# ydixon/yolo_v3

Measured on AMD Instinct MI355X. Metric: images/sec (YOLOv3 forward + decode + NMS, 416x416, bs=64 per GPU), higher is better.
Workload: dtype f32 (exact fp32 MFMA); 1 GPU; 416x416 bs=64 per GPU, 64 distinct synthetic scenes per GPU, SW-1 synthetic weights, conf=0.50 nms=0.40; global_batch=64, parallelism=dp1, entry=Detector.run_device, lanes=2

## Files before the change

### yolo_v3_amd/_ffi.py

```python
import ctypes
import os

_HERE = os.path.dirname(os.path.abspath(__file__))
LIB_PATH = (os.environ.get("YV3_LIB") if os.environ.get("YV3_MEASURE") == "1" else None) or os.path.join(_HERE, "libyv3.so")

if os.environ.get("YV3_MEASURE") != "1":
    _stray = sorted(k for k in os.environ if k.startswith("YV3_") and k not in ("YV3_MEASURE", "YV3_DIST_BACKEND", "YV3_DUMP_PLAN"))
    if _stray:
        import warnings
        warnings.warn("yolo_v3_amd: %s set but ignored -- library / kernel-selection overrides are honoured in measurement sessions only "
                      "(YV3_MEASURE=1); the bundled libyv3.so and the default plans are used" % ", ".join(_stray), RuntimeWarning)

F32, BF16, F32X3, F32H2 = 0, 1, 2, 3
BF16_ACT = 4
F16 = 5
I8 = 6
ACT_LINEAR, ACT_LEAKY = 0, 1
PP_EVAL, PP_PROB = 1, 2
OPT_NO_PINGPONG, OPT_K3S1, OPT_WINO_EVEN, OPT_WINO_ALWAYS, OPT_TWO_LANES, OPT_WINO4_TILES = 1, 2, 4, 8, 16, 32
OPT_TILE_SHIFT = 8
(TILE_AUTO, TILE_256x128_W8, TILE_128x128_W8, TILE_128x128_W4, TILE_128x64, TILE_256x128_W4, TILE_256x256, TILE_256x128_W4_ROLL,
 TILE_256x256_ROLL, TILE_256x256_ROLL4) = range(10)
TILE_192x256_ROLL, TILE_W4_192x128, TILE_256x256_PP3, TILE_256x256_PP4, TILE_192x256_PP3, TILE_192x256_PP4 = 11, 12, 13, 14, 15, 16
T0_F32_TILE_64, T0_F32_TILE_128_W4, T0_F32_TILE_128_1X1, T0_WINO2_HALF, T0_WINO2_FULL = 2, 6, 7, 8, 9
T0_WINO4_NEVER, T0_WINO4_ALWAYS, T0_GEMM_NEVER, T0_GEMM_ALWAYS = 10, 11, 13, 14
T1_WINO4_NO_EVEN, T1_WINO4_NO_FULL, T1_GEMM_ALL_ROWS = 1, 2, 3
T1P_NO_SHORT_K, T1P_WINO_OTHER_LOOP, T1P_BF16_ROUND3, T1P_BF16_NO_192, T1P_NO_W4 = 1, 2, 8, 16, 32
T1P_NO_W4_1X1, T1P_NO_W4_3X3, T1P_W4_LANES_3X3, T1P_BF16_ROLL, T1P_BF16_PP3 = 64, 128, 256, 512, 1024
KERNEL_LINE_BYTES = 96


def conv2d_kernel(desc):
    buf = ctypes.create_string_buffer(KERNEL_LINE_BYTES)
    check(lib().yv3_conv2d_kernel(ctypes.byref(desc), buf, KERNEL_LINE_BYTES), "yv3_conv2d_kernel")
    return buf.value.decode()

c_void_p, c_int, c_float, c_size_t, c_longlong = (ctypes.c_void_p, ctypes.c_int, ctypes.c_float,
                                                  ctypes.c_size_t, ctypes.c_longlong)


class ConvDesc(ctypes.Structure):
    _fields_ = [("x", c_void_p), ("x2", c_void_p), ("w", c_void_p), ("alpha", c_void_p), ("beta", c_void_p),
                ("residual", c_void_p), ("y", c_void_p),
                ("B", c_int), ("H", c_int), ("W", c_int), ("cin", c_int), ("cin_up", c_int),
                ("cout", c_int), ("cout_pad", c_int), ("k", c_int), ("stride", c_int), ("act", c_int),
                ("dtype", c_int), ("out_dtype", c_int), ("flags", c_void_p),
                ("workspace", c_void_p), ("workspace_bytes", ctypes.c_size_t),
                ("dec_out", c_void_p), ("dec_out_batch_stride", c_longlong), ("dec_stride", c_float),
                ("dec_anchors", c_float * 6), ("options", ctypes.c_uint), ("big_tile_min", c_int), ("tune", c_int * 4),
                ("x_plane_stride", c_longlong), ("x2_plane_stride", c_longlong), ("y_plane_stride", c_longlong),
                ("w_wino", c_void_p), ("alpha_wino", c_void_p), ("wino_ws", c_void_p), ("wino_ws_bytes", ctypes.c_size_t),
                ("w_wino4", c_void_p), ("s_res", c_float), ("inv_s_out", c_float)]


COCO_MAX_MAXDETS = 8
ELIMIT = -6


class CocoEvalDesc(ctypes.Structure):
    _fields_ = [("n_gt", c_int), ("n_det", c_int), ("n_img", c_int), ("n_cat", c_int),
                ("gt_img", c_void_p), ("gt_cat", c_void_p), ("gt_box", c_void_p), ("gt_area", c_void_p),
                ("gt_crowd", c_void_p), ("gt_id", c_void_p),
                ("det_img", c_void_p), ("det_cat", c_void_p), ("det_box", c_void_p), ("det_score", c_void_p),
                ("n_iou", c_int), ("n_rec", c_int), ("n_area", c_int), ("n_maxdet", c_int),
                ("iou_thrs", c_void_p), ("rec_thrs", c_void_p), ("area_rng", c_void_p),
                ("max_dets", c_int * COCO_MAX_MAXDETS),
                ("precision", c_void_p), ("recall", c_void_p), ("scores", c_void_p), ("status", c_void_p)]


YOLO_LOSS_MAX_ROWS = 1024
EINVAL, ESHAPE, EWORKSPACE = -1, -2, -3


class YoloLossDesc(ctypes.Structure):
    _fields_ = [("logits", c_void_p), ("grad", c_void_p),
                ("stride_b", c_longlong), ("stride_p", c_longlong), ("stride_c", c_longlong),
                ("target", c_void_p), ("B", c_int), ("H", c_int), ("W", c_int), ("T", c_int), ("num_class", c_int),
                ("img_dim_h", c_float), ("anchors", c_float * 18), ("mask", c_int * 3),
                ("sums", c_void_p), ("counts", c_void_p), ("status", c_void_p)]
# ... 163 lines not shown
```

### yolo_v3_amd/csrc/conv_select.cpp

```cpp
#include "conv_select.h"
#include <stdio.h>

yv3_conv_shape yv3_conv_out_shape(const yv3_conv_desc* d) {
    const int pad = (d->k - 1) / 2;
    yv3_conv_shape s;
    s.Ho = (d->H + 2 * pad - d->k) / d->stride + 1;
    s.Wo = (d->W + 2 * pad - d->k) / d->stride + 1;
    s.M = (long long)d->B * s.Ho * s.Wo;
    return s;
}


static bool planes_wino_rule(const yv3_conv_desc* d, int np, long long ncu) {
    const int npad = d->cout_pad;
    const bool k3 = d->k == 3, dual = d->cin_up > 0, out_f32 = d->out_dtype == YV3_F32;
    if (!(d->w_wino && np == 2 && k3 && d->stride == 1 && !out_f32 && !dual && d->alpha_wino && npad % 128 == 0 &&
          d->x_plane_stride <= 0 && d->y_plane_stride <= 0)) return false;
    const long long tiles = (((long long)d->B * ((d->H + 1) / 2) * ((d->W + 1) / 2) + 127) / 128) * (npad / 128);
    if (d->options & YV3_OPT_WINO_ALWAYS) return true;
#ifndef YV3_AB_NO_TWO_LANES_RULE
    if (d->options & YV3_OPT_TWO_LANES) return tiles * 100 >= 27 * ncu;
#endif
    if (tiles * 100 <= 105 * ncu) return tiles * 100 >= 62 * ncu;
    return tiles * 100 >= 75 * ((tiles + ncu - 1) / ncu) * ncu;
// ... 125 lines not shown
    if (P > 1 && (8 * ((tail + 7) / 8) * P > YV3_SEL_WINO4_MAX_TAIL_WG || (lone_only && W > ncu))) return -1;
    const long long f = W <= ncu ? 1 : W <= 2 * ncu ? 2 : 2 * ((W + 2 * ncu - 1) / (2 * ncu));
    return (6 / P) * nkx * f + (P > 1 ? 29 + 5 * P : 0);
}
static void wino4_schedule(const yv3_conv_desc* d, long long items, int ncu, int* n_full, int* parts) {
    const int slots = 2 * ncu;
    *n_full = (int)items; *parts = 1;
    if ((d->options & YV3_OPT_WINO4_TILES) || d->tune[1] == YV3_T1_WINO4_NO_EVEN || items < 1) return;
    const long long full = d->tune[1] == YV3_T1_WINO4_NO_FULL ? 0 : (items / slots) * slots;
    const long long tail = items - full;
    if (tail == 0) return;
    const int nkx = 6 * (d->cin / 32);
    int best = 1; long long best_cost = wino4_tail_cost(tail, 1, nkx, ncu, false);
    for (int P = 2; P <= 6; ++P) {
        if (6 % P) continue;
        const long long cost = wino4_tail_cost(tail, P, nkx, ncu, full > 0);
        if (cost >= 0 && cost < best_cost) { best = P; best_cost = cost; }
    }
    if ((d->tune[2] == 2 || d->tune[2] == 3 || d->tune[2] == 6) && wino4_tail_cost(tail, d->tune[2], nkx, ncu, false) >= 0) best = d->tune[2];
    if (best == 1) return;
    *n_full = (int)full; *parts = best;
}

static bool wino4_pays(const yv3_conv_desc* d, long long items, long long ncu) {
    if ((d->options & YV3_OPT_WINO4_TILES) || d->tune[1] == YV3_T1_WINO4_NO_EVEN) return items * 10 >= 3 * ncu;
    return d->cin >= 256 ? true : d->cin == 128 ? items * 100 >= 17 * ncu : items * 100 >= 39 * ncu;
}

yv3_f32_choice yv3_select_f32(const yv3_conv_desc* d, int ncu_) {
    yv3_f32_choice c = {};
    c.form = YV3_FORM_DIRECT; c.launches = 1; c.parts = 1;
    const auto fail = [&c](int rc) { c.rc = rc; return c; };
    const auto pick = [&c](yv3_f32_kernel k, int ntiles) { c.kernel = k; c.ntiles = ntiles; return c; };
    const long long ncu = ncu_;
    const bool k3 = d->k == 3, dual = d->cin_up > 0;
    const int tune0 = d->tune[0];
    const yv3_conv_shape sh = yv3_conv_out_shape(d);
    const long long M = sh.M;
    if (M > 0x7fffffffLL) return fail(YV3_ESHAPE);
    c.Ho = sh.Ho; c.Wo = sh.Wo; c.M = (int)M;
    c.pin = !(d->options & YV3_OPT_TWO_LANES);

    if (d->w_wino4 && d->wino_ws && k3 && d->stride == 1 && !dual && d->cout % YV3_SEL_WINO4_CHANNELS == 0 && (d->cin == 64 || d->cin % 128 == 0) &&
        d->cout_pad == d->cout && d->alpha && tune0 != YV3_T0_WINO4_NEVER) {
        const long long T = (long long)d->B * ((d->H + 3) / 4) * ((d->W + 3) / 4);
        const long long items = ((T + YV3_SEL_WINO4_TILES - 1) / YV3_SEL_WINO4_TILES) * (d->cout / YV3_SEL_WINO4_CHANNELS);
        if ((d->options & YV3_OPT_WINO_ALWAYS) || tune0 == YV3_T0_WINO4_ALWAYS || wino4_pays(d, items, ncu)) {
            if (d->wino_ws_bytes < yv3_wino4_ws_bytes(d->B, d->H, d->W, d->cin)) return fail(YV3_EWORKSPACE);
            const unsigned long long vb = 36ull * T * d->cin * 4, ub = 36ull * d->cout * d->cin * 4;
            if (vb > 0xffffffffull || ub > 0xffffffffull) return fail(YV3_ESHAPE);
            if (items * 6 > 0x7fffffffLL) return fail(YV3_ESHAPE);
            c.form = YV3_FORM_WINOGRAD4; c.launches = 2;
            wino4_schedule(d, items, ncu_, &c.n_full, &c.parts);
            return pick(YV3_FK_WINO4, d->cout / YV3_SEL_WINO4_CHANNELS);
        }
    }

    if (d->w_wino && d->alpha_wino && k3 && d->stride == 1 && !dual && d->cout % 128 == 0 && d->cout_pad == d->cout) {
        const long long T2 = (long long)d->B * ((d->H + 1) / 2) * ((d->W + 1) / 2);
        const long long t128 = ((T2 + 127) / 128) * (d->cout / 128);
        if ((d->options & YV3_OPT_WINO_ALWAYS) || t128 * 100 >= 40 * ncu) {
            if (!d->wino_ws || d->wino_ws_bytes < (size_t)16 * T2 * d->cin * sizeof(float)) return fail(YV3_EWORKSPACE);
            c.form = YV3_FORM_WINOGRAD; c.launches = 2;
            const long long last = t128 % ncu;
            c.wino2_half = tune0 == YV3_T0_WINO2_HALF || (tune0 != YV3_T0_WINO2_FULL && ((t128 > ncu && last > 0 && 3 * last <= 2 * ncu) || 2 * t128 <= ncu));
            return pick(YV3_FK_WINO2, d->cout / 128);
        }
    }

    const int np = d->cout_pad;
    const bool g_k1 = d->k == 1 && d->stride == 1, g_k3 = k3 && d->cout % 128 == 0 && tune0 == YV3_T0_GEMM_ALWAYS;
    if ((g_k1 || g_k3) && !d->cin_up && !d->residual && d->cin % 32 == 0 && d->cout % 64 == 0 && d->cout <= 1024 && d->cout_pad == d->cout && tune0 != YV3_T0_GEMM_NEVER &&
        !((long long)d->B * d->H * d->W * d->cin * 4 > 0xfffffe00LL || M * d->cout * 4 > 0xffffffffLL || (long long)d->cout * d->cin * d->k * d->k * 4 > 0xffffffffLL)) {
        const bool wide = d->cout % 128 == 0;
        const int bm = (wide ? 2 : 4) * YV3_SEL_GEMM_WAVE_M, bn = (wide ? 4 : 2) * YV3_SEL_GEMM_WAVE_N, ntn = d->cout / bn;
        const long long mt = (M + bm - 1) / bm;
        if (tune0 == YV3_T0_GEMM_ALWAYS || mt * ntn >= ncu) {
            long long mt_run = mt;
            if (d->tune[1] != YV3_T1_GEMM_ALL_ROWS) {
                const long long rounds = mt * ntn / ncu, rest = mt * ntn - rounds * ncu;
                if (rounds >= 1 && rest > 0 && 2 * rest <= ncu) mt_run = rounds * ncu / ntn;
            }
            c.gemm_rows = (int)(mt_run * bm < M ? mt_run * bm : M);
            const long long tiles = ((c.gemm_rows + bm - 1) / bm) * ntn;
            c.gemm_grid = (int)(tiles < ncu ? (tiles + 7) / 8 * 8 : ncu);
            if (c.gemm_rows < M) {
                c.launches = 2;
                c.rest = k3 ? YV3_FK_128x128_W8 : np % 128 == 0 ? YV3_FK_64x64 : YV3_FK_128x64;
                c.rest_ntiles = k3 ? np / 128 : np / 64;
            }
            return pick(k3 ? YV3_FK_GEMM_K3 : wide ? YV3_FK_GEMM_128x128 : YV3_FK_GEMM_256x64, ntn);
        }
    }

    if (np % 128 == 0) {
        const long long blocks128 = ((M + 127) / 128) * (np / 128);
        if (blocks128 >= 384 && tune0 == YV3_T0_F32_TILE_128_W4) return pick(YV3_FK_128x128_W4, np / 128);
        if (blocks128 >= 384 && tune0 != YV3_T0_F32_TILE_64 && (k3 || tune0 == YV3_T0_F32_TILE_128_1X1)) return pick(YV3_FK_128x128_W8, np / 128);
        return pick(YV3_FK_64x64, np / 64);
    }
    if (np % 64 == 0) return pick(YV3_FK_128x64, np / 64);
    return pick(YV3_FK_128x32, np / 32);
}


const char* yv3_planes_kernel_name(yv3_planes_kernel k) {
// ... 58 lines not shown
```

### yolo_v3_amd/csrc/conv_select.h

```cpp
#pragma once
#include <stddef.h>
#include "yv3.h"

enum {
    YV3_TILE_AUTO = 0,
    YV3_TILE_256x128_W8 = 1,
    YV3_TILE_128x128_W8 = 2,
    YV3_TILE_128x128_W4 = 3,
    YV3_TILE_128x64 = 4,
    YV3_TILE_256x128_W4 = 5,
    YV3_TILE_256x256 = 6,
    YV3_TILE_256x128_W4_ROLL = 7,
    YV3_TILE_256x256_ROLL = 8,
    YV3_TILE_256x256_ROLL4 = 9,
    YV3_TILE_192x256_ROLL = 11,
    YV3_TILE_W4_192x128 = 12,
    YV3_TILE_256x256_PP3 = 13,
    YV3_TILE_256x256_PP4 = 14,
    YV3_TILE_192x256_PP3 = 15,
    YV3_TILE_192x256_PP4 = 16,
};
enum {
    YV3_T0_F32_TILE_64 = 2,
    YV3_T0_F32_TILE_128_W4 = 6,
    YV3_T0_F32_TILE_128_1X1 = 7,
    YV3_T0_WINO2_HALF = 8,
    YV3_T0_WINO2_FULL = 9,
    YV3_T0_WINO4_NEVER = 10,
    YV3_T0_WINO4_ALWAYS = 11,
    YV3_T0_GEMM_NEVER = 13,
    YV3_T0_GEMM_ALWAYS = 14,
};
enum {
    YV3_T1_WINO4_NO_EVEN = 1,
    YV3_T1_WINO4_NO_FULL = 2,
    YV3_T1_GEMM_ALL_ROWS = 3,
};
enum {
    YV3_T1P_NO_SHORT_K = 1,
    YV3_T1P_WINO_OTHER_LOOP = 2,
    YV3_T1P_BF16_ROUND3 = 8,
    YV3_T1P_BF16_NO_192 = 16,
    YV3_T1P_NO_W4 = 32,
    YV3_T1P_NO_W4_1X1 = 64,
    YV3_T1P_NO_W4_3X3 = 128,
    YV3_T1P_W4_LANES_3X3 = 256,
    YV3_T1P_BF16_ROLL = 512,
    YV3_T1P_BF16_PP3 = 1024,
};

constexpr int YV3_SEL_CHUNK = 32;
constexpr int YV3_SEL_W4_BM = 192, YV3_SEL_W4_BN = 128;
constexpr int YV3_SEL_GEMM_WAVE_M = 64, YV3_SEL_GEMM_WAVE_N = 32;
constexpr int YV3_SEL_WINO4_TILES = 32, YV3_SEL_WINO4_CHANNELS = 64;

#define YV3_SK_MAX_WG 512
#define YV3_SK_PART_BYTES (512 * 64 * 4)
static inline size_t yv3_sk_bytes() { return (size_t)YV3_SK_MAX_WG * (YV3_SK_PART_BYTES + sizeof(int)); }
#define YV3_WINO_SK_MAX_WG 512
#define YV3_WINO_SK_PART_BYTES (512 * 128 * 4)
static inline size_t yv3_wino_sk_bytes() { return (size_t)YV3_WINO_SK_MAX_WG * (YV3_WINO_SK_PART_BYTES + sizeof(int)) + 256; }
constexpr int YV3_SEL_WINO4_MAX_TAIL_WG = 2 * YV3_WINO_SK_MAX_WG - 1;
static inline size_t yv3_wino4_v_bytes(int B, int H, int W, int cin) { return (size_t)36 * B * ((H + 3) / 4) * ((W + 3) / 4) * cin * sizeof(float); }
static inline size_t yv3_wino4_ws_bytes(int B, int H, int W, int cin) { return ((yv3_wino4_v_bytes(B, H, W, cin) + 255) & ~(size_t)255) + yv3_wino_sk_bytes(); }

enum yv3_planes_kernel {
    YV3_PK_256x128_W8,
    YV3_PK_128x128_W8,
    YV3_PK_128x128_W4,
    YV3_PK_128x64,
    YV3_PK_128x32,
    YV3_PK_256x128_W8_PP6,
    YV3_PK_256x128_W4,
    YV3_PK_256x128_W4_ROLL,
    YV3_PK_256x256,
    YV3_PK_256x256_ROLL,
    YV3_PK_256x256_ROLL4,
    YV3_PK_256x256_PP3,
    YV3_PK_256x256_PP4,
    YV3_PK_192x256_ROLL,
    YV3_PK_192x256_PP3,
    YV3_PK_192x256_PP4,
    YV3_PK_W4_192x128,
    YV3_PK_K3S1_256x128,
    YV3_PK_K3S1_128x128,
    YV3_PK_K3S1_128x64,
    YV3_PK_WINO_PINGPONG,
    YV3_PK_WINO_ROLL,
    YV3_PK_WINO_EVEN,
};
const char* yv3_planes_kernel_name(yv3_planes_kernel k);
enum yv3_planes_loop {
    YV3_LOOP_PLAIN,
    YV3_LOOP_ROLLING,
    YV3_LOOP_PINGPONG,
};
const char* yv3_planes_loop_name(yv3_planes_loop l);
struct yv3_planes_choice {
    int rc;
    int form, launches;
    yv3_planes_kernel kernel;
    int Ho, Wo, M;
    int ntiles;
    yv3_planes_loop loop;
    bool stream_k;
    int grid;
};

enum yv3_f32_kernel {
    YV3_FK_NONE,
    YV3_FK_128x128_W8, YV3_FK_128x128_W4, YV3_FK_64x64, YV3_FK_128x64, YV3_FK_128x32,
    YV3_FK_WINO2,
    YV3_FK_WINO4,
    YV3_FK_GEMM_128x128, YV3_FK_GEMM_256x64, YV3_FK_GEMM_K3,
};
const char* yv3_f32_kernel_name(yv3_f32_kernel k);
struct yv3_f32_choice {
    int rc;
    int form, launches;
    yv3_f32_kernel kernel;
    int Ho, Wo, M;
    int ntiles;
    bool pin;
    bool wino2_half;
    int n_full, parts;
    int gemm_rows;
    int gemm_grid;
    yv3_f32_kernel rest;
    int rest_ntiles;
};

struct yv3_conv_shape { int Ho, Wo; long long M; };
yv3_conv_shape yv3_conv_out_shape(const yv3_conv_desc* d);

yv3_planes_choice yv3_select_planes(const yv3_conv_desc* d, int np, int ncu);
yv3_planes_choice yv3_select_planes_i8(const yv3_conv_desc* d, int ncu);
yv3_f32_choice yv3_select_f32(const yv3_conv_desc* d, int ncu);

constexpr size_t YV3_KERNEL_LINE_BYTES = 96;
int yv3_describe_planes(const yv3_planes_choice& c, char* buf, size_t buf_bytes);
int yv3_describe_f32(const yv3_f32_choice& c, char* buf, size_t buf_bytes);
```

### yolo_v3_amd/csrc/conv_wino4_f32.hip

```cpp
#include <type_traits>
#include "yv3_common.h"

namespace {

#define W4F_GPTR(p) ((const __attribute__((address_space(1))) void*)(p))
#define W4F_LPTR(p) ((__attribute__((address_space(3))) void*)(p))

typedef float f32x2 __attribute__((ext_vector_type(2)));

constexpr int BNC = 64;
constexpr int BMT = 32;
constexpr int ROWB = 128;
constexpr int U_BYTES = BNC * ROWB;
constexpr int V_BYTES = BMT * ROWB;
constexpr int STAGE = U_BYTES + V_BYTES;
#define W4F_NSTAGE 4
#ifndef W4F_PRIO
#define W4F_PRIO 3
#endif
#ifndef W4F_EXTRA_LDS
#define W4F_EXTRA_LDS 0
#endif
#ifndef W4F_DMA_FIRST
#define W4F_DMA_FIRST 0
#endif
constexpr int NSTAGE = W4F_NSTAGE;
#if defined(YV3_MEASURE) && defined(W4F_ABL)
constexpr int ABL = W4F_ABL;
#else
constexpr int ABL = 0;
#endif

struct Wino4Params {
    const float* v;
    const float* u;
    const float* alpha;
    const float* beta;
    const float* res;
    float* y;
    int C, Cout, H, W, th, tw, T;
    int cchunks;
    int nblk_n;
    int act;
    long long pos_stride;
    unsigned u_bytes, v_bytes;
    int nitems, n_full, parts;
    float* sk_parts;
    int* sk_flags;
    int* status;
};
constexpr int W4F_MAX_TAIL_WG = 2 * YV3_WINO_SK_MAX_WG - 1;
constexpr int W4F_PART_FLOATS = 4 * 32 * 256;

template <int N> __device__ __forceinline__ void w4f_wait_vmcnt() { asm volatile("s_waitcnt vmcnt(%0)" :: "n"(N) : "memory"); }

__device__ __forceinline__ int w4f_swz(int row) { return (row >> 1) & 7; }

__device__ __forceinline__ void bt_apply(const f32x4 (&d)[6], f32x4 (&o)[6]) {
    o[0] = d[0] - 1.5f * d[1] - 2.0f * d[2] + 1.5f * d[3] + d[4];
    o[1] = 0.5f * d[2] - d[1] + 2.5f * d[3] + d[4];
    o[2] = d[1] - 2.5f * d[2] + 0.5f * d[3] + d[4];
    o[3] = 2.0f * (d[3] - d[1]) - d[2] + d[4];
    o[4] = 0.5f * (d[1] - d[3]) - d[2] + d[4];
    o[5] = d[1] - 1.5f * d[2] - 2.0f * d[3] + 1.5f * d[4] + d[5];
}

__global__ __launch_bounds__(256) void wino4_input_f32_kernel(const float* __restrict__ x, float* __restrict__ v,
                                                              int H, int W, int C, int th, int tw, long long T) {
    const int cg = C >> 2;
    const long long i = (long long)blockIdx.x * blockDim.x + threadIdx.x;
    if (i >= T * cg) return;
    const long long t = i / cg;
    const int c = (int)(i - t * cg) * 4;
    const int b = (int)(t / (th * tw));
    const int rem = (int)(t - (long long)b * th * tw);
    const int ty = rem / tw, tx = rem - ty * tw;
    const int y0 = 4 * ty - 1, x0 = 4 * tx - 1;
    f32x4 tr[6][6];
#pragma unroll
    for (int r = 0; r < 6; ++r) {
        f32x4 d[6];
        const int yy = y0 + r;
#pragma unroll
        for (int q = 0; q < 6; ++q) {
            const int xx = x0 + q;
            const bool ok = (unsigned)yy < (unsigned)H && (unsigned)xx < (unsigned)W;
            d[q] = ok ? *reinterpret_cast<const f32x4*>(x + (((long long)b * H + yy) * W + xx) * C + c) : f32x4{0.f, 0.f, 0.f, 0.f};
        }
        bt_apply(d, tr[r]);
    }
#pragma unroll
    for (int l = 0; l < 6; ++l) {
        f32x4 col[6], o[6];
#pragma unroll
        for (int r = 0; r < 6; ++r) col[r] = tr[r][l];
        bt_apply(col, o);
#pragma unroll
        for (int xi = 0; xi < 6; ++xi) *reinterpret_cast<f32x4*>(v + ((long long)(xi * 6 + l) * T + t) * C + c) = o[xi];
    }
}

__global__ __launch_bounds__(256) void wino4_pack_kernel(const float* __restrict__ u, float* __restrict__ out, int cout, int cin) {
    const long long i = (long long)blockIdx.x * blockDim.x + threadIdx.x;
    const long long n4 = (long long)cout * cin * 36 / 4;
    if (i >= n4) return;
    const int cch = cin / 32;
    const int ps = (int)(i & 7);
    const int row = (int)((i >> 3) & 63);
    long long r = i >> 9;
// ... 43 lines not shown
        const int rows = 6 / p.parts;
        xa = part * rows; xb = xa + rows;
    }

    const __amdgpu_buffer_rsrc_t urs = __builtin_amdgcn_make_buffer_rsrc(const_cast<float*>(p.u), 0, (int)p.u_bytes, 0x00020000);
    const __amdgpu_buffer_rsrc_t vrs = __builtin_amdgcn_make_buffer_rsrc(const_cast<float*>(p.v), 0, (int)p.v_bytes, 0x00020000);
    unsigned usoff = 0;
    const unsigned uoff = lane * 16;
    unsigned vsoff = 0, voff = 0;
    int pf_c = 0;
    int pf_k = 0, pf_end = 0;
    auto dma_piece = [&](int i, unsigned char* stage) {
        if (ABL & 8) return;
        if (i == 0)      __builtin_amdgcn_raw_ptr_buffer_load_lds(urs, W4F_LPTR(stage + (2 * wid) * 1024), 16, uoff, usoff, 0, 0);
        else if (i == 1) __builtin_amdgcn_raw_ptr_buffer_load_lds(urs, W4F_LPTR(stage + (2 * wid) * 1024), 16, uoff, usoff, 1024, 0);
        else             __builtin_amdgcn_raw_ptr_buffer_load_lds(vrs, W4F_LPTR(stage + U_BYTES + wid * 1024), 16, voff, vsoff, 0, 0);
    };
    auto dma_advance = [&]() {
        if (pf_k + 1 < pf_end) {
            ++pf_k;
            usoff += BNC * 32 * 4;
            vsoff += 128;
            pf_c += 32;
            if (pf_c == p.C) { pf_c = 0; vsoff += (unsigned)(p.pos_stride - p.C) * 4u; }
        }
    };

    const int fr = lane & 15, fq = lane >> 4;
    const int urow = 16 * wid + fr;
    const int u_off0 = urow * ROWB + ((fq ^ w4f_swz(urow)) << 4);
    const int u_off1 = urow * ROWB + (((4 + fq) ^ w4f_swz(urow)) << 4);
    int v_off0[2], v_off1[2];
#pragma unroll
    for (int b = 0; b < 2; ++b) {
        const int r = 16 * b + fr;
        v_off0[b] = U_BYTES + r * ROWB + ((fq ^ w4f_swz(r)) << 4);
        v_off1[b] = U_BYTES + r * ROWB + (((4 + fq) ^ w4f_swz(r)) << 4);
    }

    f32x4 P[2], R[4][2], Y[4][4][2];
    struct Frag { f32x4 ua, va0, va1, ub, vb0, vb1; };
    auto read_frag = [&](const unsigned char* st) {
        Frag f;
        if (ABL & 4) { f.ua = f.va0 = f.va1 = f.ub = f.vb0 = f.vb1 = f32x4{(float)lane, 1.f, 2.f, 3.f}; return f; }
        f.ua = *reinterpret_cast<const f32x4*>(st + u_off0);
        f.va0 = *reinterpret_cast<const f32x4*>(st + v_off0[0]);
        f.va1 = *reinterpret_cast<const f32x4*>(st + v_off0[1]);
        f.ub = *reinterpret_cast<const f32x4*>(st + u_off1);
        f.vb0 = *reinterpret_cast<const f32x4*>(st + v_off1[0]);
        f.vb1 = *reinterpret_cast<const f32x4*>(st + v_off1[1]);
        return f;
    };
    Frag F0, F1;
    using TrueT = std::integral_constant<bool, true>;
    using FalseT = std::integral_constant<bool, false>;

#if defined(YV3_MEASURE) && defined(W4F_TIMELINE)
    unsigned long long tl_t = __builtin_amdgcn_s_memtime(), tl_sync = 0, tl_burst = 0, tl_fold = 0;
    const unsigned long long tl_entry = tl_t;
#define W4F_MARK(acc_) do { const unsigned long long t_ = __builtin_amdgcn_s_memtime(); acc_ += t_ - tl_t; tl_t = t_; } while (0)
#else
#define W4F_MARK(acc_) do {} while (0)
#endif
    auto chunk = [&](auto first_c, auto stage_c, const Frag& F, Frag& G) {
        constexpr bool FIRST = decltype(first_c)::value;
        constexpr int S = decltype(stage_c)::value;
        const f32x4 zero4 = {0.f, 0.f, 0.f, 0.f};
        W4F_MARK(tl_fold);
        w4f_wait_vmcnt<3 * (NSTAGE - 2)>();
        __builtin_amdgcn_s_waitcnt(0xC07F);
        if (!(ABL & 16)) __builtin_amdgcn_s_barrier();
        __builtin_amdgcn_sched_barrier(0);
        W4F_MARK(tl_sync);
        unsigned char* const fr_ = lds + S * STAGE;
        G = read_frag(lds + ((S + 1) % NSTAGE) * STAGE);
#if W4F_PRIO == 3
        __builtin_amdgcn_s_setprio(1);
#endif
#pragma unroll
        for (int t = 0; t < 4; ++t) {
            if (ABL & 2) { P[0][t] += F.ua[t] + F.va0[t]; P[1][t] += F.va1[t]; }
            else {
            P[0] = __builtin_amdgcn_mfma_f32_16x16x4f32(F.ua[t], F.va0[t], (FIRST && t == 0) ? zero4 : P[0], 0, 0, 0);
            P[1] = __builtin_amdgcn_mfma_f32_16x16x4f32(F.ua[t], F.va1[t], (FIRST && t == 0) ? zero4 : P[1], 0, 0, 0);
            }
            __builtin_amdgcn_sched_barrier(0);
            if (t < 3) dma_piece(t, fr_);
            __builtin_amdgcn_sched_barrier(0);
        }
#pragma unroll
        for (int t = 0; t < 4; ++t) {
            if (ABL & 2) { P[0][t] += F.ub[t] + F.vb0[t]; P[1][t] += F.vb1[t]; }
            else {
            P[0] = __builtin_amdgcn_mfma_f32_16x16x4f32(F.ub[t], F.vb0[t], P[0], 0, 0, 0);
            P[1] = __builtin_amdgcn_mfma_f32_16x16x4f32(F.ub[t], F.vb1[t], P[1], 0, 0, 0);
            }
        }
#if W4F_PRIO == 3
        __builtin_amdgcn_s_setprio(0);
#endif
        dma_advance();
        W4F_MARK(tl_burst);
    };

    auto position = [&](auto nu_c) {
        constexpr int nu = decltype(nu_c)::value;
        {
            using S0 = std::integral_constant<int, 0>; using S1 = std::integral_constant<int, 1>;
            using S2 = std::integral_constant<int, 2>; using S3 = std::integral_constant<int, 3>;
            if constexpr (CCH2) {
                if constexpr ((nu & 1) == 0) { chunk(TrueT{}, S0{}, F0, F1); chunk(FalseT{}, S1{}, F1, F0); }
                else                         { chunk(TrueT{}, S2{}, F0, F1); chunk(FalseT{}, S3{}, F1, F0); }
            } else {
                chunk(TrueT{}, S0{}, F0, F1); chunk(FalseT{}, S1{}, F1, F0); chunk(FalseT{}, S2{}, F0, F1); chunk(FalseT{}, S3{}, F1, F0);
                for (int cc = 4; cc < p.cchunks; cc += 4) {
                    chunk(FalseT{}, S0{}, F0, F1); chunk(FalseT{}, S1{}, F1, F0); chunk(FalseT{}, S2{}, F0, F1); chunk(FalseT{}, S3{}, F1, F0);
                }
            }
            if (ABL & 32) return;
#pragma unroll
            for (int b = 0; b < 2; ++b) {
#pragma unroll
                for (int j = 0; j < 4; ++j) {
                    constexpr float z = 0.f;
                    const float cf = at_coef(j, nu);
                    if (cf != z) {
#pragma unroll
                        for (int e = 0; e < 4; ++e) R[j][b][e] = fmaf(P[b][e], cf, R[j][b][e]);
                    }
                }
            }
        }
    };
    {
        const int nb = item % p.nblk_n;
        const int n0 = nb * BNC;
        const int m0 = (item / p.nblk_n) * BMT;
        {
            const int k0 = xa * nkx;
            usoff = (unsigned)((((long long)nb * nk + k0) * (BNC * 32) + (2 * wid) * 256) * 4);
            const int vrow = 8 * wid + (lane >> 3);
            const int vt = min(m0 + vrow, p.T - 1);
            vsoff = (unsigned)m0 * (unsigned)p.C * 4u + (unsigned)(6 * xa) * (unsigned)p.pos_stride * 4u;
            voff = (unsigned)(vt - m0) * (unsigned)p.C * 4u + ((((unsigned)lane & 7u) ^ (unsigned)w4f_swz(vrow)) << 4);
            pf_c = 0; pf_k = k0; pf_end = xb * nkx;
        }
#pragma unroll
        for (int b = 0; b < 2; ++b) {
            P[b] = f32x4{0.f, 0.f, 0.f, 0.f};
#pragma unroll
            for (int j = 0; j < 4; ++j) {
                R[j][b] = f32x4{0.f, 0.f, 0.f, 0.f};
#pragma unroll
                for (int i = 0; i < 4; ++i) Y[i][j][b] = f32x4{0.f, 0.f, 0.f, 0.f};
            }
        }
#pragma unroll
        for (int d = 0; d < NSTAGE; ++d) {
#pragma unroll
            for (int i = 0; i < 3; ++i) dma_piece(i, lds + d * STAGE);
            dma_advance();
        }
        w4f_wait_vmcnt<3 * (NSTAGE - 1)>();
        __builtin_amdgcn_s_barrier();
#if W4F_PRIO == 1
        if (__builtin_amdgcn_s_getreg((3 << 11) | 4) & 1) __builtin_amdgcn_s_setprio(2);
#elif W4F_PRIO == 2
        if ((blockIdx.x >> 8) & 1) __builtin_amdgcn_s_setprio(2);
#endif
        F0 = read_frag(lds);
        for (int xi = xa; xi < xb; ++xi) {
            position(std::integral_constant<int, 0>{}); position(std::integral_constant<int, 1>{}); position(std::integral_constant<int, 2>{});
            position(std::integral_constant<int, 3>{}); position(std::integral_constant<int, 4>{}); position(std::integral_constant<int, 5>{});
            const float c1 = xi == 0 || xi == 5 ? 0.f : xi == 1 ? 1.f : xi == 2 ? -1.f : xi == 3 ? 0.5f : -2.f;
            const float cfi[4] = {xi == 5 ? 0.f : 1.f, c1, c1 * c1, xi == 5 ? 1.f : c1 * c1 * c1};
#pragma unroll
            for (int i = 0; i < 4; ++i) {
                if (cfi[i] == 0.f) continue;
#pragma unroll
                for (int j = 0; j < 4; ++j)
#pragma unroll
                    for (int b = 0; b < 2; ++b)
#pragma unroll
                        for (int e = 0; e < 4; ++e) Y[i][j][b][e] = fmaf(R[j][b][e], cfi[i], Y[i][j][b][e]);
            }
#pragma unroll
            for (int j = 0; j < 4; ++j)
#pragma unroll
                for (int b = 0; b < 2; ++b) R[j][b] = f32x4{0.f, 0.f, 0.f, 0.f};
        }
        w4f_wait_vmcnt<0>();
#if defined(YV3_MEASURE) && defined(W4F_TIMELINE)
        const unsigned long long tl_loop_end = __builtin_amdgcn_s_memtime();
#endif

        if constexpr (SK) {
            if (xa == 0 && xb < 6) {
                for (int k = 1; k < p.parts; ++k) {
                    const int partner = sk_t + 8 * k;
                    if (tid == 0) {
                        int n = 0, f;
                        while ((f = __hip_atomic_load(p.sk_flags + partner, __ATOMIC_RELAXED, __HIP_MEMORY_SCOPE_AGENT)) == 0 && ++n < (1 << 22))
                            __builtin_amdgcn_s_sleep(2);
                        if ((f == 0 || f != 1 + (int)(__builtin_amdgcn_s_getreg((3 << 11) | 20) & 15)) && p.status) atomicOr(p.status, 2);
                        __hip_atomic_store(p.sk_flags + partner, 0, __ATOMIC_RELAXED, __HIP_MEMORY_SCOPE_AGENT);
                    }
                    __syncthreads();
                    const float* w = p.sk_parts + (size_t)partner * W4F_PART_FLOATS + wid * (32 * 256) + lane * 4;
#pragma unroll
                    for (int i = 0; i < 4; ++i) {
                        f32x4 t[4][2];
#pragma unroll
                        for (int j = 0; j < 4; ++j)
#pragma unroll
                            for (int b = 0; b < 2; ++b) t[j][b] = *reinterpret_cast<const f32x4*>(w + ((i * 4 + j) * 2 + b) * 256);
#pragma unroll
                        for (int j = 0; j < 4; ++j)
#pragma unroll
                            for (int b = 0; b < 2; ++b) Y[i][j][b] += t[j][b];
                        __builtin_amdgcn_sched_barrier(0);
                    }
                }
            }
        }

        const bool raw = SK && xa > 0;
        const int cw = n0 + 16 * wid + 4 * fq;
        const f32x4 one4 = {1.f, 1.f, 1.f, 1.f}, zero4 = {0.f, 0.f, 0.f, 0.f};
        const f32x4 al = raw ? one4 : *reinterpret_cast<const f32x4*>(p.alpha + cw);
        const f32x4 be = raw ? zero4 : *reinterpret_cast<const f32x4*>(p.beta + cw);
        const bool leaky = !raw && p.act == YV3_ACT_LEAKY;
        const float* const res = raw ? nullptr : p.res;
        float* const ybase = raw ? p.sk_parts + (size_t)sk_t * W4F_PART_FLOATS + wid * (32 * 256) + lane * 4 : p.y;
        long long pix[2];
        int py[2], px[2];
#pragma unroll
        for (int b = 0; b < 2; ++b) {
            const int t = m0 + 16 * b + fr;
            if (t < p.T) {
                const int tt = p.th * p.tw;
                const int bi = t / tt, rem = t - bi * tt;
                const int ty = rem / p.tw, tx = rem - ty * p.tw;
                py[b] = 4 * ty; px[b] = 4 * tx;
                pix[b] = ((long long)bi * p.H + py[b]) * p.W + px[b];
            } else { pix[b] = -1; py[b] = px[b] = 0; }
        }
        auto out_off = [&](int i, int j, int b) -> long long {
            if (raw) return ((i * 4 + j) * 2 + b) * 256;
            const bool ok = pix[b] >= 0 && py[b] + i < p.H && px[b] + j < p.W;
            return ok ? (pix[b] + (long long)i * p.W + j) * p.Cout + cw : -1;
        };
        f32x4 rr[2][4][2];
        auto load_res = [&](int i) {
#pragma unroll
            for (int j = 0; j < 4; ++j)
#pragma unroll
                for (int b = 0; b < 2; ++b) {
                    const long long off = out_off(i, j, b);
                    rr[i & 1][j][b] = off >= 0 ? *reinterpret_cast<const f32x4*>(res + off) : f32x4{0.f, 0.f, 0.f, 0.f};
                }
        };
        if (res) load_res(0);
#pragma unroll
        for (int i = 0; i < ((ABL & 1) ? 1 : 4); ++i) {
            if (res && i + 1 < 4) load_res(i + 1);
#pragma unroll
            for (int j = 0; j < 4; ++j)
#pragma unroll
                for (int b = 0; b < 2; ++b) {
                    const long long off = out_off(i, j, b);
                    f32x4 q;
#pragma unroll
                    for (int e = 0; e < 4; ++e) {
                        float v = fmaf(Y[i][j][b][e], al[e], be[e]);
                        if (leaky) v = v > 0.f ? v : 0.1f * v;
                        q[e] = res ? v + rr[i & 1][j][b][e] : v;
                    }
                    if (off >= 0) *reinterpret_cast<f32x4*>(ybase + off) = q;
                }
        }
        if (raw) {
            asm volatile("s_waitcnt vmcnt(0)" ::: "memory");
            __syncthreads();
            if (tid == 0) __hip_atomic_store(p.sk_flags + sk_t, 1 + (int)(__builtin_amdgcn_s_getreg((3 << 11) | 20) & 15),
                                             __ATOMIC_RELAXED, __HIP_MEMORY_SCOPE_AGENT);
        }
#if defined(YV3_MEASURE) && defined(W4F_TIMELINE)
        if (blockIdx.x == W4F_TIMELINE && lane == 0) {
            const unsigned long long tl_end = __builtin_amdgcn_s_memtime();
            __builtin_amdgcn_s_waitcnt(0);
            float* dbg = p.y + wid * 8;
            dbg[0] = (float)tl_sync / nk; dbg[1] = (float)tl_burst / nk; dbg[2] = (float)tl_fold / nk; dbg[3] = (float)(tl_loop_end - tl_entry);
            dbg[4] = (float)(tl_end - tl_loop_end); dbg[5] = (float)nk;
        }
#endif
    }
}

}

extern "C" int yv3_pack_wino4_weight_f32(const float* u_oc66, float* packed, int cout, int cin, void* stream) {
    if (!u_oc66 || !packed || cout <= 0 || cin <= 0) return YV3_EINVAL;
    if (cout % 64 || (cin != 64 && cin % 128)) return YV3_ESHAPE;
    const long long n4 = (long long)cout * cin * 9;
    hipLaunchKernelGGL(wino4_pack_kernel, dim3((unsigned)((n4 + 255) / 256)), dim3(256), 0, (hipStream_t)stream, u_oc66, packed, cout, cin);
    YV3_CHECK_LAUNCH();
    return 0;
}

static_assert(BMT == YV3_SEL_WINO4_TILES && BNC == YV3_SEL_WINO4_CHANNELS && W4F_MAX_TAIL_WG == YV3_SEL_WINO4_MAX_TAIL_WG && ROWB == 4 * YV3_SEL_CHUNK,
              "conv_select.cpp counts this kernel's items, tail workgroups and chunks");

extern "C" size_t yv3_wino4_workspace_bytes(int B, int H, int W, int cin) {
    if (B <= 0 || H <= 0 || W <= 0 || cin <= 0) return 0;
    return yv3_wino4_ws_bytes(B, H, W, cin);
}

int yv3_conv2d_wino4_f32(const yv3_conv_desc* d, const yv3_f32_choice& c, hipStream_t s) {
    const int th = (d->H + 3) / 4, tw = (d->W + 3) / 4;
    const long long T = (long long)d->B * th * tw;
    float* v = (float*)d->wino_ws;
    {
        const long long n = T * (d->cin >> 2);
        hipLaunchKernelGGL(wino4_input_f32_kernel, dim3((unsigned)((n + 255) / 256)), dim3(256), 0, s, (const float*)d->x, v, d->H, d->W, d->cin, th, tw, T);
        YV3_CHECK_LAUNCH();
    }
    Wino4Params p;
    p.v = v; p.u = (const float*)d->w_wino4;
    p.alpha = d->alpha; p.beta = d->beta; p.res = (const float*)d->residual; p.y = (float*)d->y;
    p.C = d->cin; p.Cout = d->cout; p.H = d->H; p.W = d->W; p.th = th; p.tw = tw; p.T = (int)T;
    p.cchunks = d->cin / 32; p.nblk_n = c.ntiles; p.act = d->act;
    p.pos_stride = T * d->cin;
    p.u_bytes = (unsigned)(36ull * d->cout * d->cin * 4); p.v_bytes = (unsigned)(36ull * T * d->cin * 4);
    const long long items = ((T + BMT - 1) / BMT) * p.nblk_n;
    p.nitems = (int)items;
    p.n_full = c.n_full; p.parts = c.parts;
    char* area = (char*)d->wino_ws + ((d->wino_ws_bytes - yv3_wino_sk_bytes()) & ~(size_t)255);
    p.sk_parts = (float*)area;
    p.sk_flags = (int*)(area + (size_t)W4F_MAX_TAIL_WG * W4F_PART_FLOATS * sizeof(float));
    p.status = d->flags;
    const size_t lds = (size_t)NSTAGE * STAGE + W4F_EXTRA_LDS;
    if (p.parts > 1) {
        const long long tail = items - p.n_full;
        const dim3 grid((unsigned)(p.n_full + 8 * ((tail + 7) / 8) * p.parts));
        if (p.cchunks == 2) hipLaunchKernelGGL((conv_wino4_f32_kernel<true, true>), grid, dim3(256), lds, s, p);
        else                hipLaunchKernelGGL((conv_wino4_f32_kernel<false, true>), grid, dim3(256), lds, s, p);
    } else {
        const dim3 grid((unsigned)items);
        if (p.cchunks == 2) hipLaunchKernelGGL((conv_wino4_f32_kernel<true, false>), grid, dim3(256), lds, s, p);
        else                hipLaunchKernelGGL((conv_wino4_f32_kernel<false, false>), grid, dim3(256), lds, s, p);
    }
    YV3_CHECK_LAUNCH();
    return 0;
}
```

Baseline: 3345 images/sec.

## Overlap Winograd-4 output rows 0-2 epilogue with last row's MFMA loop

In the F(4x4,3x3) fp32 Winograd kernel, the first three output rows are finished after the fifth transform row. Their scale, leaky and residual epilogue is then interleaved, through buffer loads and stores, into the MFMA chunks of the last inverse-transform row, leaving only row 3 for the serial epilogue. Per-lane output offsets and masks plus alpha/beta are staged in extra LDS, and vmcnt waits are recomputed at compile time to account for the extra in-flight memory ops. This only applies to small-cin layers whose output fits in 32-bit offsets. It adds LDS use, register pressure and waitcnt complexity.

Measured after the change: 3343 images/sec, median of 2. About the same (-0.0%).

```diff
diff --git a/yolo_v3_amd/_ffi.py b/yolo_v3_amd/_ffi.py
--- a/yolo_v3_amd/_ffi.py
+++ b/yolo_v3_amd/_ffi.py
@@ -24,7 +24,7 @@
 TILE_192x256_ROLL, TILE_W4_192x128, TILE_256x256_PP3, TILE_256x256_PP4, TILE_192x256_PP3, TILE_192x256_PP4 = 11, 12, 13, 14, 15, 16
 T0_F32_TILE_64, T0_F32_TILE_128_W4, T0_F32_TILE_128_1X1, T0_WINO2_HALF, T0_WINO2_FULL = 2, 6, 7, 8, 9
 T0_WINO4_NEVER, T0_WINO4_ALWAYS, T0_GEMM_NEVER, T0_GEMM_ALWAYS = 10, 11, 13, 14
-T1_WINO4_NO_EVEN, T1_WINO4_NO_FULL, T1_GEMM_ALL_ROWS = 1, 2, 3
+T1_WINO4_NO_EVEN, T1_WINO4_NO_FULL, T1_GEMM_ALL_ROWS, T1_WINO4_LATE_ROWS = 1, 2, 3, 4
 T1P_NO_SHORT_K, T1P_WINO_OTHER_LOOP, T1P_BF16_ROUND3, T1P_BF16_NO_192, T1P_NO_W4 = 1, 2, 8, 16, 32
 T1P_NO_W4_1X1, T1P_NO_W4_3X3, T1P_W4_LANES_3X3, T1P_BF16_ROLL, T1P_BF16_PP3 = 64, 128, 256, 512, 1024
 KERNEL_LINE_BYTES = 96
diff --git a/yolo_v3_amd/csrc/conv_select.cpp b/yolo_v3_amd/csrc/conv_select.cpp
--- a/yolo_v3_amd/csrc/conv_select.cpp
+++ b/yolo_v3_amd/csrc/conv_select.cpp
@@ -201,6 +201,7 @@
             if (items * 6 > 0x7fffffffLL) return fail(YV3_ESHAPE);
             c.form = YV3_FORM_WINOGRAD4; c.launches = 2;
             wino4_schedule(d, items, ncu_, &c.n_full, &c.parts);
+            c.late_rows = d->tune[1] == YV3_T1_WINO4_LATE_ROWS || M * d->cout * 4 > 0x7fffffffLL || d->cin > 4 * YV3_SEL_CHUNK;
             return pick(YV3_FK_WINO4, d->cout / YV3_SEL_WINO4_CHANNELS);
         }
     }
diff --git a/yolo_v3_amd/csrc/conv_select.h b/yolo_v3_amd/csrc/conv_select.h
--- a/yolo_v3_amd/csrc/conv_select.h
+++ b/yolo_v3_amd/csrc/conv_select.h
@@ -35,6 +35,7 @@
     YV3_T1_WINO4_NO_EVEN = 1,
     YV3_T1_WINO4_NO_FULL = 2,
     YV3_T1_GEMM_ALL_ROWS = 3,
+    YV3_T1_WINO4_LATE_ROWS = 4,
 };
 enum {
     YV3_T1P_NO_SHORT_K = 1,
@@ -124,6 +125,7 @@
     bool pin;
     bool wino2_half;
     int n_full, parts;
+    bool late_rows;
     int gemm_rows;
     int gemm_grid;
     yv3_f32_kernel rest;
diff --git a/yolo_v3_amd/csrc/conv_wino4_f32.hip b/yolo_v3_amd/csrc/conv_wino4_f32.hip
--- a/yolo_v3_amd/csrc/conv_wino4_f32.hip
+++ b/yolo_v3_amd/csrc/conv_wino4_f32.hip
@@ -7,6 +7,7 @@
 #define W4F_LPTR(p) ((__attribute__((address_space(3))) void*)(p))
 
 typedef float f32x2 __attribute__((ext_vector_type(2)));
+typedef unsigned u32x4 __attribute__((ext_vector_type(4)));
 
 constexpr int BNC = 64;
 constexpr int BMT = 32;
@@ -48,6 +49,8 @@
     float* sk_parts;
     int* sk_flags;
     int* status;
+    unsigned y_bytes;
+    int early;
 };
 constexpr int W4F_MAX_TAIL_WG = 2 * YV3_WINO_SK_MAX_WG - 1;
 constexpr int W4F_PART_FLOATS = 4 * 32 * 256;
@@ -55,6 +58,39 @@
 template <int N> __device__ __forceinline__ void w4f_wait_vmcnt() { asm volatile("s_waitcnt vmcnt(%0)" :: "n"(N) : "memory"); }
 
 __device__ __forceinline__ int w4f_swz(int row) { return (row >> 1) & 7; }
+
+constexpr int W4F_EOUT = 24;
+constexpr int W4F_EARLY_LDS = 2 * BNC * 4 + 3 * 256 * 4;
+constexpr int w4f_e_first(int V, int L) { return V == 0 ? 2 * L : L; }
+constexpr int w4f_e_num(int V, int L) { return L < 0 ? 0 : V == 0 ? 2 : 1; }
+constexpr int w4f_e_chunk(int V, int o) { return V == 0 ? o / 2 : o; }
+constexpr int w4f_e_ops(int V, int L, bool res) {
+    if (L < 0) return L == -1 && res ? 2 : 0;
+    int n = 0;
+    for (int o = w4f_e_first(V, L); o < w4f_e_first(V, L) + w4f_e_num(V, L); ++o) n += 1 + (res && o + 2 < W4F_EOUT ? 1 : 0);
+    return n;
+}
+constexpr int w4f_ring_extra(int V, int L, bool res) { return w4f_e_ops(V, L - 1, res) + w4f_e_ops(V, L - 2, res) + w4f_e_ops(V, L - 3, res); }
+constexpr int w4f_res_wait(int V, int o) {
+    int n = 0, L0 = -1;
+    if (o < 2) n += 1 - o;
+    else {
+        L0 = w4f_e_chunk(V, o - 2);
+        for (int q = o - 1; q < w4f_e_first(V, L0) + w4f_e_num(V, L0); ++q) n += q + 2 < W4F_EOUT ? 1 : 0;
+    }
+    const int L1 = w4f_e_chunk(V, o);
+    for (int L = L0 + 1; L <= L1; ++L) {
+        n += 3;
+        for (int q = w4f_e_first(V, L); q < w4f_e_first(V, L) + w4f_e_num(V, L) && !(L == L1 && q >= o); ++q) n += q + 2 < W4F_EOUT ? 1 : 0;
+    }
+    return n;
+}
+static_assert(w4f_ring_extra(0, 0, true) == 2 && w4f_ring_extra(0, 3, true) == 12 && w4f_ring_extra(0, 3, false) == 6 && w4f_ring_extra(1, 2, true) == 6 &&
+              w4f_ring_extra(1, 2, false) == 2 && w4f_ring_extra(1, 24 - 1, true) == 5,
+              "stores and residual requests of the last three chunks");
+static_assert(w4f_res_wait(0, 0) == 4 && w4f_res_wait(0, 1) == 4 && w4f_res_wait(0, 6) == 4 && w4f_res_wait(0, 7) == 4 && w4f_res_wait(1, 0) == 4 &&
+              w4f_res_wait(1, 1) == 7 && w4f_res_wait(1, 5) == 7 && w4f_res_wait(1, 23) == 6,
+              "loads behind a residual request");
 
 __device__ __forceinline__ void bt_apply(const f32x4 (&d)[6], f32x4 (&o)[6]) {
     o[0] = d[0] - 1.5f * d[1] - 2.0f * d[2] + 1.5f * d[3] + d[4];
@@ -204,6 +240,12 @@
         return f;
     };
     Frag F0, F1;
+    const bool early = p.early && (!SK || (int)blockIdx.x < p.n_full);
+    const bool eres = p.res != nullptr, eleaky = p.act == YV3_ACT_LEAKY;
+    const __amdgpu_buffer_rsrc_t yrs = __builtin_amdgcn_make_buffer_rsrc(p.y, 0, (int)p.y_bytes, 0x00020000);
+    const __amdgpu_buffer_rsrc_t rrs = __builtin_amdgcn_make_buffer_rsrc(const_cast<float*>(p.res), 0, (int)p.y_bytes, 0x00020000);
+    unsigned ebase[2], eout;
+    f32x4 eal, ebe, err[2];
     using TrueT = std::integral_constant<bool, true>;
     using FalseT = std::integral_constant<bool, false>;
 
@@ -214,12 +256,16 @@
 #else
 #define W4F_MARK(acc_) do {} while (0)
 #endif
-    auto chunk = [&](auto first_c, auto stage_c, const Frag& F, Frag& G) {
+    auto chunk_x = [&](auto first_c, auto stage_c, auto xr_c, auto xn_c, const Frag& F, Frag& G, auto extra) {
         constexpr bool FIRST = decltype(first_c)::value;
         constexpr int S = decltype(stage_c)::value;
+        constexpr int XR = decltype(xr_c)::value, XN = decltype(xn_c)::value;
+        constexpr bool EARLY = !std::is_same<decltype(extra), std::nullptr_t>::value;
         const f32x4 zero4 = {0.f, 0.f, 0.f, 0.f};
         W4F_MARK(tl_fold);
-        w4f_wait_vmcnt<3 * (NSTAGE - 2)>();
+        if constexpr (XR == XN) w4f_wait_vmcnt<3 * (NSTAGE - 2) + XN>();
+        else if (eres) w4f_wait_vmcnt<3 * (NSTAGE - 2) + XR>();
+        else w4f_wait_vmcnt<3 * (NSTAGE - 2) + XN>();
         __builtin_amdgcn_s_waitcnt(0xC07F);
         if (!(ABL & 16)) __builtin_amdgcn_s_barrier();
         __builtin_amdgcn_sched_barrier(0);
@@ -247,12 +293,63 @@
             P[0] = __builtin_amdgcn_mfma_f32_16x16x4f32(F.ub[t], F.vb0[t], P[0], 0, 0, 0);
             P[1] = __builtin_amdgcn_mfma_f32_16x16x4f32(F.ub[t], F.vb1[t], P[1], 0, 0, 0);
             }
+            if constexpr (EARLY) {
+                __builtin_amdgcn_sched_barrier(0);
+                if (t == 0) extra(std::integral_constant<int, 0>{});
+                if (t == 1) extra(std::integral_constant<int, 1>{});
+                __builtin_amdgcn_sched_barrier(0);
+            }
         }
 #if W4F_PRIO == 3
         __builtin_amdgcn_s_setprio(0);
 #endif
         dma_advance();
         W4F_MARK(tl_burst);
+    };
+    auto chunk = [&](auto first_c, auto stage_c, const Frag& F, Frag& G) {
+        chunk_x(first_c, stage_c, std::integral_constant<int, 0>{}, std::integral_constant<int, 0>{}, F, G, nullptr);
+    };
+
+    auto fold_position = [&](auto nu_c) {
+        constexpr int nu = decltype(nu_c)::value;
+        if (ABL & 32) return;
+#pragma unroll
+        for (int b = 0; b < 2; ++b) {
+#pragma unroll
+            for (int j = 0; j < 4; ++j) {
+                constexpr float z = 0.f;
+                const float cf = at_coef(j, nu);
+                if (cf != z) {
+#pragma unroll
+                    for (int e = 0; e < 4; ++e) R[j][b][e] = fmaf(P[b][e], cf, R[j][b][e]);
+                }
+            }
+        }
+    };
+    auto early_voff = [&](int o) { return ebase[o & 1] | ((eout << (31 - (16 * (o & 1) + (o >> 1)))) & 0x80000000u); };
+    auto early_soff = [&](int o) { return (unsigned)(((o >> 3) * p.W + ((o >> 1) & 3)) * p.Cout) * 4u; };
+    auto early_req = [&](auto o_c) {
+        constexpr int o = decltype(o_c)::value;
+        f32x4& r = err[o & 1];
+        const unsigned vo = early_voff(o), so = early_soff(o);
+        const __amdgpu_buffer_rsrc_t rs = rrs;
+        asm volatile("s_nop 4\n\tbuffer_load_dwordx4 %0, %1, %2, %3 offen" : "=v"(r) : "v"(vo), "s"(rs), "s"(so) : "memory");
+    };
+    auto early_out = [&](auto o_c, auto v_c) {
+        constexpr int o = decltype(o_c)::value, V = decltype(v_c)::value;
+        constexpr int b = o & 1, i = o >> 3, j = (o >> 1) & 3;
+        f32x4& r = err[b];
+        if (eres) asm volatile("s_waitcnt vmcnt(%1)" : "+v"(r) : "n"(w4f_res_wait(V, o)) : "memory");
+#pragma unroll
+        for (int e = 0; e < 4; ++e) {
+            float v = fmaf(Y[i][j][b][e], eal[e], ebe[e]);
+            if (eleaky) v = v > 0.f ? v : 0.1f * v;
+            r[e] = eres ? v + r[e] : v;
+        }
+        __builtin_amdgcn_raw_buffer_store_b128(__builtin_bit_cast(u32x4, r), yrs, early_voff(o), early_soff(o), 0);
+        if constexpr (o + 2 < W4F_EOUT) {
+            if (eres) early_req(std::integral_constant<int, o + 2>{});
+        }
     };
 
     auto position = [&](auto nu_c) {
@@ -269,20 +366,53 @@
                     chunk(FalseT{}, S0{}, F0, F1); chunk(FalseT{}, S1{}, F1, F0); chunk(FalseT{}, S2{}, F0, F1); chunk(FalseT{}, S3{}, F1, F0);
                 }
             }
-            if (ABL & 32) return;
-#pragma unroll
-            for (int b = 0; b < 2; ++b) {
-#pragma unroll
-                for (int j = 0; j < 4; ++j) {
-                    constexpr float z = 0.f;
-                    const float cf = at_coef(j, nu);
-                    if (cf != z) {
-#pragma unroll
-                        for (int e = 0; e < 4; ++e) R[j][b][e] = fmaf(P[b][e], cf, R[j][b][e]);
-                    }
-                }
-            }
-        }
+            fold_position(nu_c);
+        }
+    };
+    auto position5 = [&](auto nu_c, auto v_c) {
+        constexpr int nu = decltype(nu_c)::value, V = decltype(v_c)::value;
+        using S0 = std::integral_constant<int, 0>; using S1 = std::integral_constant<int, 1>;
+        using S2 = std::integral_constant<int, 2>; using S3 = std::integral_constant<int, 3>;
+        auto chunk5 = [&](auto first_c, auto stage_c, auto l_c, const Frag& F, Frag& G) {
+            constexpr int L = decltype(l_c)::value;
+            chunk_x(first_c, stage_c, std::integral_constant<int, w4f_ring_extra(V, L, true)>{}, std::integral_constant<int, w4f_ring_extra(V, L, false)>{}, F, G,
+                    [&](auto t_c) {
+                        constexpr int t = decltype(t_c)::value;
+                        if constexpr (t < w4f_e_num(V, L)) early_out(std::integral_constant<int, w4f_e_first(V, L) + t>{}, v_c);
+                    });
+        };
+#define W4F_L(n_) std::integral_constant<int, (n_)>{}
+        if constexpr (V == 0) {
+            if constexpr ((nu & 1) == 0) { chunk5(TrueT{}, S0{}, W4F_L(2 * nu), F0, F1); chunk5(FalseT{}, S1{}, W4F_L(2 * nu + 1), F1, F0); }
+            else                         { chunk5(TrueT{}, S2{}, W4F_L(2 * nu), F0, F1); chunk5(FalseT{}, S3{}, W4F_L(2 * nu + 1), F1, F0); }
+        } else {
+            constexpr int L0 = 4 * nu;
+            chunk5(TrueT{}, S0{}, W4F_L(L0), F0, F1); chunk5(FalseT{}, S1{}, W4F_L(L0 + 1), F1, F0);
+            chunk5(FalseT{}, S2{}, W4F_L(L0 + 2), F0, F1); chunk5(FalseT{}, S3{}, W4F_L(L0 + 3), F1, F0);
+        }
+#undef W4F_L
+        fold_position(nu_c);
+#pragma unroll
+        for (int j = 0; j < 4; ++j)
+#pragma unroll
+            for (int b = 0; b < 2; ++b) { f32x4& rj = R[j][b]; asm volatile("" : "+v"(rj)); }
+    };
+    auto row5 = [&](auto v_c) {
+        {
+            const float* const eab = reinterpret_cast<const float*>(lds + NSTAGE * STAGE) + 16 * wid + 4 * fq;
+            const unsigned* const elane = reinterpret_cast<const unsigned*>(lds + NSTAGE * STAGE + 2 * BNC * 4) + tid;
+            eal = *reinterpret_cast<const f32x4*>(eab); ebe = *reinterpret_cast<const f32x4*>(eab + BNC);
+            ebase[0] = elane[0]; ebase[1] = elane[256]; eout = elane[512];
+        }
+        if (eres) { early_req(std::integral_constant<int, 0>{}); early_req(std::integral_constant<int, 1>{}); }
+        position5(std::integral_constant<int, 0>{}, v_c); position5(std::integral_constant<int, 1>{}, v_c); position5(std::integral_constant<int, 2>{}, v_c);
+        position5(std::integral_constant<int, 3>{}, v_c); position5(std::integral_constant<int, 4>{}, v_c); position5(std::integral_constant<int, 5>{}, v_c);
+#pragma unroll
+        for (int j = 0; j < 4; ++j)
+#pragma unroll
+            for (int b = 0; b < 2; ++b)
+#pragma unroll
+                for (int e = 0; e < 4; ++e) Y[3][j][b][e] = fmaf(R[j][b][e], 1.f, Y[3][j][b][e]);
     };
     {
         const int nb = item % p.nblk_n;
@@ -297,6 +427,28 @@
             voff = (unsigned)(vt - m0) * (unsigned)p.C * 4u + ((((unsigned)lane & 7u) ^ (unsigned)w4f_swz(vrow)) << 4);
             pf_c = 0; pf_k = k0; pf_end = xb * nkx;
         }
+        if (early) {
+            float* const eab = reinterpret_cast<float*>(lds + NSTAGE * STAGE);
+            unsigned* const elane = reinterpret_cast<unsigned*>(lds + NSTAGE * STAGE + 2 * BNC * 4);
+            if (tid < 2 * BNC) eab[tid] = tid < BNC ? p.alpha[n0 + tid] : p.beta[n0 + tid - BNC];
+            const int cw = n0 + 16 * wid + 4 * fq;
+            unsigned out = ~0u;
+#pragma unroll
+            for (int b = 0; b < 2; ++b) {
+                const int t = m0 + 16 * b + fr;
+                unsigned base = 0u;
+                if (t < p.T) {
+                    const int tt = p.th * p.tw;
+                    const int bi = t / tt, rem = t - bi * tt;
+                    const int ty = rem / p.tw, tx = rem - ty * p.tw;
+                    base = (unsigned)((((long long)bi * p.H + 4 * ty) * p.W + 4 * tx) * p.Cout + cw) * 4u;
+                    const unsigned cols = (1u << min(4, p.W - 4 * tx)) - 1u, rows = 0x111u & ((1u << 4 * min(3, p.H - 4 * ty)) - 1u);
+                    out &= ~((cols * rows) << (16 * b));
+                }
+                elane[b * 256 + tid] = base;
+            }
+            elane[2 * 256 + tid] = out;
+        }
 #pragma unroll
         for (int b = 0; b < 2; ++b) {
             P[b] = f32x4{0.f, 0.f, 0.f, 0.f};
@@ -321,7 +473,7 @@
         if ((blockIdx.x >> 8) & 1) __builtin_amdgcn_s_setprio(2);
 #endif
         F0 = read_frag(lds);
-        for (int xi = xa; xi < xb; ++xi) {
+        for (int xi = xa; xi < (early ? 5 : xb); ++xi) {
             position(std::integral_constant<int, 0>{}); position(std::integral_constant<int, 1>{}); position(std::integral_constant<int, 2>{});
             position(std::integral_constant<int, 3>{}); position(std::integral_constant<int, 4>{}); position(std::integral_constant<int, 5>{});
             const float c1 = xi == 0 || xi == 5 ? 0.f : xi == 1 ? 1.f : xi == 2 ? -1.f : xi == 3 ? 0.5f : -2.f;
@@ -340,6 +492,10 @@
             for (int j = 0; j < 4; ++j)
 #pragma unroll
                 for (int b = 0; b < 2; ++b) R[j][b] = f32x4{0.f, 0.f, 0.f, 0.f};
+        }
+        if (early) {
+            if constexpr (CCH2) row5(std::integral_constant<int, 0>{});
+            else row5(std::integral_constant<int, 1>{});
         }
         w4f_wait_vmcnt<0>();
 #if defined(YV3_MEASURE) && defined(W4F_TIMELINE)
@@ -412,10 +568,12 @@
                     rr[i & 1][j][b] = off >= 0 ? *reinterpret_cast<const f32x4*>(res + off) : f32x4{0.f, 0.f, 0.f, 0.f};
                 }
         };
-        if (res) load_res(0);
+        if (res && !early) load_res(0);
 #pragma unroll
         for (int i = 0; i < ((ABL & 1) ? 1 : 4); ++i) {
+            if (early && i < 3) continue;
             if (res && i + 1 < 4) load_res(i + 1);
+            if (res && early && i == 3) load_res(3);
 #pragma unroll
             for (int j = 0; j < 4; ++j)
 #pragma unroll
@@ -491,7 +649,9 @@
     p.sk_parts = (float*)area;
     p.sk_flags = (int*)(area + (size_t)W4F_MAX_TAIL_WG * W4F_PART_FLOATS * sizeof(float));
     p.status = d->flags;
-    const size_t lds = (size_t)NSTAGE * STAGE + W4F_EXTRA_LDS;
+    p.early = !c.late_rows;
+    p.y_bytes = c.late_rows ? 0u : (unsigned)((long long)d->B * d->H * d->W * d->cout * 4);
+    const size_t lds = (size_t)NSTAGE * STAGE + W4F_EARLY_LDS + W4F_EXTRA_LDS;
     if (p.parts > 1) {
         const long long tail = items - p.n_full;
         const dim3 grid((unsigned)(p.n_full + 8 * ((tail + 7) / 8) * p.parts));
```
